# guodashun/peg-in-hole-gym

Hardware: AMD Instinct MI355X
Metric: env-steps/sec (higher is better)
Workload: dtype f32

## Files before the change

### include/pih.h

```cpp
#ifndef PIH_H
#define PIH_H
#include <stdint.h>
#ifdef __cplusplus
extern "C" {
#endif

#define PIH_ABI_VERSION 4
#define PIH_STATE_WORDS 256
#define PIH_ACTION_DIM 4
#define PIH_OBS_DIM 5
#define PIH_DEBUG_WORDS 1024

enum {
  PIH_DBG_UDOT = 0,
  PIH_DBG_NCONTACT = 38,
  PIH_DBG_PGS_ITERS = 39,
  PIH_DBG_CONTACT = 40,
  PIH_DBG_CONTACT_STRIDE = 12,
  PIH_DBG_CONTACT_KEY = 10,
  PIH_DBG_CONTACT_LAMBDA = 11,
  PIH_DBG_DINV = 640,
  PIH_DBG_FLY_UDOT = 0,
  PIH_DBG_FLY_NCONTACT = 12,
  PIH_DBG_FLY_PGS_ITERS = 13,
  PIH_DBG_FLY_LIMIT_ROWS = 14,
  PIH_DBG_FLY_CAND = 16,
  PIH_DBG_FLY_CAND_STRIDE = 10,
  PIH_DBG_FLY_LAMBDA = 200,
  PIH_DBG_CYCLES = 900,
  PIH_DBG_T_START = 940,
  PIH_DBG_T_END = 943,
  PIH_DBG_HW_ID = 946,
  PIH_DBG_XCC_ID = 947
};

enum {
// ... 117 lines not shown
```

### peg_in_hole_gym_amd/_lib.py

```python
import ctypes as C
import os

_HERE = os.path.dirname(os.path.abspath(__file__))
LIB_PATH = os.environ.get("PIH_LIB_PATH") or os.path.join(_HERE, "csrc", "libpih_hip.so")

ABI_VERSION = 4
STATE_WORDS, DEBUG_WORDS, ACTION_DIM, OBS_DIM = 256, 1024, 4, 5
FLY_STATE_WORDS, FLY_ACTION_DIM, FLY_OBS_DIM = 48, 6, 6
CAM_WORDS = 13
FLY_CAM_DEFAULT = (1.6, 0.0, 1.2, 0.0, 0.0, 0.2, 0.0, 0.0, 1.0, 60.0, 1.0, 0.01, 100.0)
RENDER_SHADED, RENDER_CAM_EE = 1, 2
RENDER_OUT_RGBA8, RENDER_OUT_DEPTH, RENDER_CAM_DEVICE = 4, 8, 16
SEG_OBJECT, SEG_TABLE, SEG_NONE = 6, 7, 255
RENDER_CAM_EE_POS = 32
VIEW_SEG_HOLE, VIEW_SEG_TABLE, VIEW_SEG_PIPE0 = 9, 10, 32
VIEW_CAM_WRIST = (0.0, 0.0, 0.0, 0.0, 0.0, -10.0, 0.0, 1.0, 0.0, 60.0, 1.0, 0.001, 1000.0)
VIEW_CAM_OVERVIEW = (1.33, -0.02, 1.05, 0.05, -0.25, 0.3, 0.0, 0.0, 1.0, 40.0, 1.0, 0.01, 100.0)
LIGHT_WORDS = 11
LIGHT_DEFAULT = (-50.0, 30.0, 100.0, 1.0, 1.0, 1.0, 0.6, 0.35, 0.05, 2.0, 0.8)
RENDER_LIGHT_DEVICE = 64
FIELD_STATE, FIELD_TIP_POSE, FIELD_CONTACT_FORCE, FIELD_DEBUG, FIELD_EE_POS = 0, 1, 2, 3, 4
TASK_PEG_IN_HOLE, TASK_RANDOM_FLY = 0, 1
S_QARM, S_QDARM, S_POS, S_QUAT, S_VLIN, S_VANG, S_QJ, S_QDJ, S_TARGET = 0, 9, 18, 21, 25, 28, 31, 54, 77
S_FSM, S_FSMT, S_DONE, S_GRASP, S_RANDY, S_RNG_HI, S_RNG, S_STEPS, S_OFFSET = 86, 87, 88, 89, 90, 91, 92, 93, 94
S_SPARE, S_TIP, S_CFORCE, S_NCONTACT, S_PGS_ITERS, S_EE, S_GRASP_ANGLE, S_INVALID, S_ATTACH_QZ, S_SOLVER = 97, 98, 105, 106, 107, 108, 111, 112, 113, 114
S_CACHE_N, S_CACHE_KEY, S_CACHE_LAMBDA = 128, 129, 177
F_Q, F_QD, F_TARGET, F_OPOS, F_OQUAT, F_OVLIN, F_OVANG, F_DONE, F_STEPS, F_RNG, F_RNG_HI, F_OFFSET, F_SPARE, F_INVALID, F_EE, F_CFORCE, F_NCONTACT = \
    0, 6, 12, 18, 21, 25, 28, 31, 32, 33, 34, 35, 38, 39, 40, 43, 44
DBG_UDOT, DBG_NCONTACT, DBG_PGS_ITERS, DBG_CONTACT, DBG_CONTACT_STRIDE, DBG_CONTACT_KEY, DBG_CONTACT_LAMBDA, DBG_DINV = 0, 38, 39, 40, 12, 10, 11, 640
DBG_FLY_UDOT, DBG_FLY_NCONTACT, DBG_FLY_PGS_ITERS, DBG_FLY_LIMIT_ROWS, DBG_FLY_CAND, DBG_FLY_CAND_STRIDE, DBG_FLY_LAMBDA = 0, 12, 13, 14, 16, 10, 200
DBG_CYCLES, DBG_T_START, DBG_T_END, DBG_HW_ID, DBG_XCC_ID = 900, 940, 943, 946, 947

EXPORTS = ["pih_default_config", "pih_abi_version", "pih_task_dims", "pih_object_name", "pih_create", "pih_destroy", "pih_reset", "pih_reseed", "pih_step", "pih_step_n",
           "pih_get_state", "pih_set_state", "pih_ik", "pih_ik_ur5", "pih_render", "pih_render_ex", "pih_render_cam", "pih_grasp_labels", "pih_timing", "pih_timing2", "pih_set_timing", "pih_last_error"]
LIGHT_EXPORTS = ["pih_render_lit"]
VIEW_EXPORTS = ["pih_render_view"]


class PihConfig(C.Structure):
    _fields_ = [("n_envs", C.c_int32), ("env_index0", C.c_int32), ("mode", C.c_int32), ("solver_iters", C.c_int32),
                ("ik_iters", C.c_int32), ("max_episode_steps", C.c_int32), ("auto_reset", C.c_int32),
                ("enable_self_collision", C.c_int32), ("debug", C.c_int32), ("schedule", C.c_int32), ("enable_arm_collision", C.c_int32), ("task_id", C.c_int32), ("solver_path", C.c_int32), ("attach_ball", C.c_int32), ("exit_check_stride", C.c_int32), ("object_id", C.c_int32), ("seed", C.c_uint64),
                ("dt", C.c_float), ("residual_threshold", C.c_float), ("erp", C.c_float), ("warmstart", C.c_float),
                ("contact_margin", C.c_float), ("linear_slop", C.c_float), ("ik_damping", C.c_float), ("ik_residual", C.c_float),
# ... 79 lines not shown
```

### peg_in_hole_gym_amd/csrc/pih_common.h

```cpp
#pragma once
#include <string.h>
#include "../../include/pih.h"
#include "../../include/pih_model.h"
#include "pih_math.h"

namespace pih {

constexpr int NL = PIH_NL, ANL = PIH_ARM_NL, ONL = PIH_OBJ_NL, ND = PIH_NDOF;
constexpr int NSAMP = PIH_PIPE_NSAMP;
constexpr int CMAX = 48;
constexpr int CAMAX = 12;
constexpr int CL = 20;
constexpr int NROWC = 3 * CMAX;
constexpr int WPS = 39;
constexpr int WMS = 31;
constexpr int NMOT = 32;
constexpr int NLIM = 18;
static_assert(PIH_DBG_UDOT + ND <= PIH_DBG_NCONTACT && PIH_DBG_CONTACT + PIH_DBG_CONTACT_STRIDE * CMAX <= PIH_DBG_DINV &&
              PIH_DBG_DINV + 3 * CMAX <= PIH_DBG_CYCLES && PIH_DBG_XCC_ID < PIH_DEBUG_WORDS, "debug words of the peg-in-hole step (include/pih.h PIH_DBG_*) overlap");

PIH_CONST int L_PARENT[NL] = PIH_LINK_PARENT;
PIH_CONST int L_JTYPE[NL] = PIH_LINK_JTYPE;
PIH_CONST real L_RFIX[NL][9] = PIH_LINK_RFIX;
PIH_CONST real L_TFIX[NL][3] = PIH_LINK_TFIX;
PIH_CONST real L_AXIS[NL][3] = PIH_LINK_AXIS;
PIH_CONST real L_MASS[NL] = PIH_LINK_MASS;
PIH_CONST real L_COM[NL][3] = PIH_LINK_COM;
PIH_CONST real L_INERTIA[NL][6] = PIH_LINK_INERTIA;
PIH_CONST real L_LO[NL] = PIH_LINK_LO;
PIH_CONST real L_HI[NL] = PIH_LINK_HI;
PIH_CONST real L_DAMPING[NL] = PIH_LINK_DAMPING;
PIH_CONST real L_MU[NL] = PIH_LINK_MU;
PIH_CONST real ARM_BASE_R[9] = PIH_ARM_BASE_R;
namespace model_ce {
// ... 54 lines not shown
};

inline void config_defaults(pih_config* c) {
  memset(c, 0, sizeof *c);
  c->n_envs = 1; c->env_index0 = 0; c->mode = 0; c->solver_iters = 50; c->ik_iters = 20; c->max_episode_steps = 2227; c->auto_reset = 0;
  c->enable_self_collision = 1; c->enable_arm_collision = 3; c->task_id = PIH_TASK_PEG_IN_HOLE; c->debug = 0; c->schedule = 1; c->exit_check_stride = 16;
  c->seed = 0; c->dt = 1.0f / 240.0f; c->residual_threshold = 1e-7f; c->erp = 0.2f; c->warmstart = 0.85f; c->contact_margin = 0.005f;
  c->linear_slop = 1e-5f; c->ik_damping = 0.5f; c->ik_residual = 1e-4f; c->dv = 2.0f / 240.0f;
}
inline Params params_from_config(const pih_config* c) {
  Params P;
  P.dt = (real)c->dt; P.resid = (real)c->residual_threshold; P.erp = (real)c->erp; P.warm = (real)c->warmstart; P.margin = (real)c->contact_margin;
  P.slop = (real)c->linear_slop; P.ikdamp = (real)c->ik_damping; P.ikres = (real)c->ik_residual; P.dv = (real)c->dv;
  P.iters = c->solver_iters; P.ikiters = c->ik_iters; P.mode = c->mode; P.maxsteps = c->max_episode_steps; P.autoreset = c->auto_reset;
  P.selfcol = c->enable_self_collision; P.armcol = c->enable_arm_collision; P.debug = c->debug; P.env0 = c->env_index0; P.seed = c->seed;
  P.pgsmode = c->solver_path; P.attachball = c->attach_ball; P.noprio = (c->schedule & 4) != 0; P.nospec = (c->schedule & 64) != 0;
  P.checkstride = c->exit_check_stride < 1 ? 1 : c->exit_check_stride; P.object = c->object_id;
  return P;
}

template <bool DOUBLED = true, class FC, class FN> PIH_HD int pgs_iteration_loop(int iters, int stride, FC checked, FN unchecked) {
  int it = 0;
  const int lead = stride <= 1 ? iters : 4;
  while (it < iters && it < lead) { it++; if (checked()) return it; }
  while (it < iters) {
    const int stop = it + stride - 1 < iters - 1 ? it + stride - 1 : iters - 1;
    if (DOUBLED) {
      while (it < stop) {
        it++; unchecked();
        if (it >= stop) break;
        it++; unchecked();
// ... 837 lines not shown
```

### peg_in_hole_gym_amd/csrc/pih_fly.h

```cpp
#pragma once
#include <type_traits>
#include "pih_common.h"

namespace pih {
namespace fly {

constexpr int NJ = 6, FND = 12, NS = PIH_FLY_OBJ_MAXSPH;
constexpr int NA = 5;
constexpr int NC = 2 * NS + NA;
constexpr int SW = PIH_FLY_STATE_WORDS;
static_assert(PIH_DBG_FLY_UDOT + FND <= PIH_DBG_FLY_NCONTACT && PIH_DBG_FLY_CAND + PIH_DBG_FLY_CAND_STRIDE * NC <= PIH_DBG_FLY_LAMBDA &&
              PIH_DBG_FLY_LAMBDA + NC <= PIH_DBG_CYCLES, "debug words of the random-fly step (include/pih.h PIH_DBG_FLY_*) overlap");
constexpr int CW = 24;
enum : int {
  FC_J = 0,
  FC_W = 6,
  FC_N = 12,
  FC_RXN = 15,
  FC_IRXN = 18,
  FC_DINV = 21,
  FC_RHS = 22,
  FC_LAM = 23,
};
static_assert(FC_W == FC_J + NJ && FC_N == FC_W + NJ && FC_LAM + 1 == CW, "contact row record of the lane layout");
// ... 372 lines not shown
    stamp(4);
    real du[FND], lam_m[NJ], lam_lo[NJ], lam_hi[NJ], wjj[NJ];
    real du3[3], Wq[NJ][3];
#pragma unroll
    for (int j = 0; j < NJ; j++) {
      wjj[j] = Wm[j][j];
#pragma unroll
      for (int k = 0; k < 3; k++) {
        if constexpr (Q::QUAD) Wq[j][k] = quad.lane4() == 0 ? Wm[j][k] : quad.lane4() == 1 ? Wm[j][3 + k] : (real)0;
      }
    }
    const real LIMIT_REACH = (real)0.25;
    int limmask = 0;
#pragma unroll
    for (int j = 0; j < NJ; j++) if (q[j] - U_LO[j] < LIMIT_REACH || U_HI[j] - q[j] < LIMIT_REACH) limmask |= 1 << j;
    limmask = P.nospec ? (1 << NJ) - 1 : quad.wave_or(limmask);
    real viol = -1, vlo[NJ], vhi[NJ];
    auto joint_tot = [&](auto JTAG, real duj, auto CHECKTAG, real& worst) __attribute__((always_inline)) -> real {
      constexpr int j = decltype(JTAG)::value;
      constexpr bool CHECK = decltype(CHECKTAG)::value;
      const real lim = U_EFFORT[j] * dt, di = mdi[j];
      real dl = mrhs[j] - duj * di, sum = med3_(lam_m[j] + dl, -lim, lim);
      dl = sum - lam_m[j]; lam_m[j] = sum;
      if (CHECK) { const real v = dl * dl - P.resid * di * di; worst = v > worst ? v : worst; }
      real dj = duj + dl * wjj[j], tot = dl;
      viol = max_(viol, max_(vlo[j] - dj, dj - vhi[j]));
      if (__builtin_expect(((limmask >> j) & 1) != 0, 0)) {
        const real r2 = lrl[j] - dj * di;
        real s2 = max_(lam_lo[j] + r2, (real)0);
        const real d2 = s2 - lam_lo[j]; lam_lo[j] = s2; tot += d2; dj += d2 * wjj[j];
        if (CHECK) { const real v = d2 * d2 - P.resid * di * di; worst = v > worst ? v : worst; }
// ... 181 lines not shown
```

### peg_in_hole_gym_amd/csrc/pih_hip.hip

```cpp
#include <hip/hip_runtime.h>
#include <dlfcn.h>
#include <cstdio>
#include <cstring>
#include <string>
#include <vector>
#include "pih_device.h"
#include "pih_render.h"
#include "pih_fly.h"
#include "pih_fly_render.h"

using namespace pih;

namespace pih {
void fly_image_launch(int fmt, dim3 grid, hipStream_t stream, const float* state, void* out, const fly::FlyCam& cam, const float* cam_dev,
                      int n, int object, int env_begin, int W, int H, int rows_per_strip, int flags);
void view_launch(int fmt, dim3 grid, hipStream_t stream, const float* state, void* out, const fly::FlyCam& cam, const float* cam_dev,
                 int env_begin, int W, int H, int rows_per_strip, int flags);
int lit_light_check(const float* words, const char** what);
void lit_launch(bool fly_task, int fmt, dim3 grid, hipStream_t stream, const float* state, void* out, const fly::FlyCam& cam, const float* cam_dev,
                const float* light, const float* light_dev, int n, int object, int env_begin, int W, int H, int rows_per_strip, int flags);
}

constexpr int PRE_THREADS = 256;
__device__ __forceinline__ int contact_bin(float ncontact) {
// ... 561 lines not shown
      HIPCHK(h, hipMemset(h->bins, 0, 3 * h->bin_ints * sizeof(int)));
    }
  } else if (cfg->schedule & 1) HIPCHK(h, hipMalloc(&h->order, (size_t)cfg->n_envs * sizeof(int)));
  hipLaunchKernelGGL(pih_init_offsets_kernel, dim3((cfg->n_envs + 63) / 64), dim3(64), 0, 0, h->state, *offd, cfg->n_envs);
  hipLaunchKernelGGL(pih_reset_kernel, dim3(cfg->n_envs), dim3(64), 0, 0, h->P, h->state, (const unsigned char*)nullptr, 0, 0);
  if (h->bins) hipLaunchKernelGGL(pih_bins_init_kernel, dim3(64), dim3(256), 0, 0, h->state, h->bins + h->bin_ints, cfg->n_envs);
  HIPCHK(h, hipGetLastError());
  HIPCHK(h, hipDeviceSynchronize());
  return 0;
}

int pih_create(const pih_config* cfg, const float* offsets_host, pih_handle** out) {
  if (!cfg || !out || cfg->n_envs <= 0) { g_err = "pih_create: bad arguments"; return -2; }
  if (cfg->task_id != PIH_TASK_PEG_IN_HOLE && cfg->task_id != PIH_TASK_RANDOM_FLY) { g_err = "pih_create: unknown task_id"; return -2; }
  if (cfg->task_id == PIH_TASK_RANDOM_FLY && (cfg->object_id < 0 || cfg->object_id >= PIH_FLY_NOBJ)) { g_err = "pih_create: unknown object_id for the random-fly task"; return -2; }
  if ((cfg->schedule & 3) >= 2 || (cfg->schedule & ~(3 | 4 | 8 | 32 | 64)) != 0) {
    g_err = "pih_create: schedule = " + std::to_string(cfg->schedule) + " is not supported (0 or 1, plus any of 4, 8, 32, 64)";
    return -2;
  }
  int ndev = 0;
  hipError_t e = hipGetDeviceCount(&ndev);
  if (e != hipSuccess || ndev == 0) { g_err = "pih_create: no HIP device (this library has no CPU path)"; return -3; }
  pih_handle* h = new pih_handle;
  h->cfg = *cfg; h->P = params_from_config(cfg);
  h->fly = cfg->task_id == PIH_TASK_RANDOM_FLY; h->words = h->fly ? PIH_FLY_STATE_WORDS : PIH_STATE_WORDS;
  float* offd = nullptr;
  int rc = -1;
  if (hipGetDevice(&h->device) == hipSuccess) rc = create_impl(h, offsets_host, &offd);
  else g_err = "pih_create: hipGetDevice failed";
  if (offd) hipFree(offd);
  if (rc != 0) { pih_destroy(h); return rc; }
  *out = h;
// ... 325 lines not shown
```

### peg_in_hole_gym_amd/csrc/pih_step.h

```cpp
#pragma once

namespace pih {

template <class W> PIH_HD void aba(W& w, Shared& sh) {
  w.stamp(15);
  link_velocities(w, sh);
  w.stamp(8);
  w.par(NL, [&](int L) {
    int p = L_PARENT[L], jt = L_JTYPE[L];
    real m = L_MASS[L];
    V3 rc = ld3(sh.a.LRC[L]); S3 Ic = lds3(sh.a.LIC[L]);
    V3 wv = ld3(sh.VW[L]), vv = ld3(sh.VV[L]);
    real* I = sh.a.IAP[L];
    real r2 = dot(rc, rc);
    I[0] = Ic.xx + m * (r2 - rc.x * rc.x); I[1] = Ic.yy + m * (r2 - rc.y * rc.y); I[2] = Ic.zz + m * (r2 - rc.z * rc.z);
    I[3] = Ic.xy - m * rc.x * rc.y; I[4] = Ic.xz - m * rc.x * rc.z; I[5] = Ic.yz - m * rc.y * rc.z;
    I[6] = 0; I[7] = -m * rc.z; I[8] = m * rc.y; I[9] = m * rc.z; I[10] = 0; I[11] = -m * rc.x; I[12] = -m * rc.y; I[13] = m * rc.x; I[14] = 0;
    I[15] = m; I[16] = m; I[17] = m; I[18] = 0; I[19] = 0; I[20] = 0;
    V3 ca = mk(0, 0, 0), cl = mk(0, 0, 0), r = mk(0, 0, 0);
    if (jt != PIH_JT_FLOATING && p >= 0) {
      V3 wp = ld3(sh.VW[p]); r = ld3(sh.LO[L]) - ld3(sh.LO[p]);
      V3 aq = sh.u[link_dof(L)] * ld3(sh.LA[L]);
      cl = cross(wp, cross(wp, r));
      if (jt == PIH_JT_REVOLUTE) ca = cross(wp, aq); else cl = cl + (real)2 * cross(wp, aq);
// ... 48 lines not shown
      if (k == ANL - 3) arm6 = na;
    }
    for (int L = 2 * ANL + 1; L < NL; L++) {
      const OC c = np_c;
      if (L + 1 < NL) np_c = oconst(L + 1);
      pipe = olink(L, pipe, c);
    }
  }
}

template <class W>
PIH_HD void step_env(W& w, Shared& sh, const Params& P, const Ovf& ov, int env, const real* action, real* obs, real* reward, unsigned char* done, real* dbg) {
  real* S = sh.S;
  const real dt = P.dt;
  w.phase_begin();
  bool frozen = !P.autoreset && S[PIH_S_DONE] != 0;
  fk_all(w, sh);
  w.phase(0);
  if (!frozen) {
    if constexpr (W::controller_inline) controller_targets(S, P, action);
    const bool ctrl_early = P.mode != 0;
    if (ctrl_early) { w.await_controller(sh); controller_rows(w, sh, P); }
    else controller_rows(w, sh, P, 1);
    w.phase(1);
    collide(w, sh, P);
    w.priority(sh.nc);
    w.phase(2);
    w.par(ND, [&](int d) {
      real v;
      if (d < 9) v = S[PIH_S_QDARM + d]; else if (d < 12) v = S[PIH_S_VLIN + d - 9]; else if (d < 15) v = S[PIH_S_VANG + d - 12]; else v = S[PIH_S_QDJ + d - 15];
// ... 87 lines not shown
```

### peg_in_hole_gym_amd/csrc/pih_wave.h

```cpp
#pragma once
#include <type_traits>
#include "pih_common.h"
#include "pih_mailbox.h"

namespace pih {

PIH_HD void debug_store_time(real* dbg, int at, long long t) { dbg[at] = (real)(t & 0xFFFF); dbg[at + 1] = (real)((t >> 16) & 0xFFFF); dbg[at + 2] = (real)((t >> 32) & 0xFFFF); }
PIH_HD void debug_store_hw_id(real* dbg) { dbg[PIH_DBG_HW_ID] = (real)(__builtin_amdgcn_s_getreg((15 << 11) | 4) & 0xFFFF); dbg[PIH_DBG_XCC_ID] = (real)__builtin_amdgcn_s_getreg((3 << 11) | 20); }

struct Wave {
  int l;
  int counter;
  static constexpr bool controller_inline = false;
  real* dbg = nullptr; int dbgmode = 0; long long t0 = 0, t1 = 0;
  PIH_HD void stamp(int k) { if (dbg && dbgmode == 2) { long long t = __builtin_readcyclecounter(); if (l == 0) dbg[PIH_DBG_CYCLES + k] = (real)(t - t0); t0 = t; } }
  PIH_HD void trace(int at, long long t) { if (l != 0) return; debug_store_time(dbg, at, t); if (at == PIH_DBG_T_START) debug_store_hw_id(dbg); }
  PIH_HD void phase_begin() { if (dbg && dbgmode == 2) { t1 = __builtin_readcyclecounter(); trace(PIH_DBG_T_START, (long long)__builtin_amdgcn_s_memrealtime()); } }
  PIH_HD void phase(int k) { if (dbg && dbgmode == 2) { long long t = __builtin_readcyclecounter(); if (l == 0) dbg[PIH_DBG_CYCLES + k] = (real)(t - t1); t1 = t; if (k == 7) trace(PIH_DBG_T_END, (long long)__builtin_amdgcn_s_memrealtime()); } }
  PIH_HD int lane() const { return l; }
  bool prio_on = true;
  PIH_HD void priority(int contacts) {
    if (!prio_on) return;
    if (contacts > 20) __builtin_amdgcn_s_setprio(3);
    else if (contacts > 14) __builtin_amdgcn_s_setprio(2);
// ... 46 lines not shown
  __asm__ volatile("v_max_f32 %0, %6, %7\n\tv_sub_f32 %1, %0, %3\n\tv_readlane_b32 %2, %0, %9\n\tv_readlane_b32 s100, %1, %9\n\t"
                   "s_lshl_b64 %4, 1, %9\n\tv_cndmask_b32_e64 %3, %3, %0, %4\n\tv_pk_fma_f32 %5, s[100:101], %8, %5 op_sel_hi:[0,1,1]"
                   : "=&v"(cand), "=&v"(dl), "=&s"(s0), "+v"(lam), "=&s"(m), "+v"(zz) : "v"(z), "v"(lo), "v"(col), "n"(G) : "scc", "s100", "s101");
}
PIH_HD void gs_row2_bounded(pk2& zz, real z, pk2 col, real hi, real& lam, int G, real& dl) {
  real cand; unsigned long long m;
  __asm__ volatile("v_med3_f32 %0, %5, -%6, %6\n\tv_sub_f32 %1, %0, %2\n\ts_lshl_b64 %3, 1, %8\n\tv_readlane_b32 s100, %1, %8\n\t"
                   "v_cndmask_b32_e64 %2, %2, %0, %3\n\ts_nop 0\n\tv_pk_fma_f32 %4, s[100:101], %7, %4 op_sel_hi:[0,1,1]"
                   : "=&v"(cand), "=&v"(dl), "+v"(lam), "=&s"(m), "+v"(zz) : "v"(z), "v"(hi), "v"(col), "n"(G) : "scc", "s100", "s101");
}
PIH_HD void gs_row2_friction(pk2& zz, real z, pk2 col, real h, real& lam, int G, real& dl) {
  real cand; unsigned long long m;
  __asm__ volatile("v_med3_f32 %0, %5, -%6, %6\n\tv_sub_f32 %1, %0, %2\n\ts_lshl_b64 %3, 1, %8\n\tv_readlane_b32 s100, %1, %8\n\t"
                   "v_cndmask_b32_e64 %2, %2, %0, %3\n\ts_nop 0\n\tv_pk_fma_f32 %4, s[100:101], %7, %4 op_sel_hi:[0,1,1]"
                   : "=&v"(cand), "=&v"(dl), "+v"(lam), "=&s"(m), "+v"(zz) : "v"(z), "v"(h), "v"(col), "n"(G) : "scc", "s100", "s101");
}
PIH_HD void gs_row1_normal(real& z, real b, real lo, real& lam, int G, real& dl, real& s0) {
  real cand, sdl; unsigned long long m;
  __asm__ volatile("v_max_f32 %0, %6, %7\n\tv_sub_f32 %1, %0, %4\n\tv_readlane_b32 %3, %0, %9\n\tv_readlane_b32 %2, %1, %9\n\t"
                   "s_lshl_b64 %5, 1, %9\n\tv_cndmask_b32_e64 %4, %4, %0, %5\n\tv_fmac_f32 %6, %2, %8"
                   : "=&v"(cand), "=&v"(dl), "=&s"(sdl), "=&s"(s0), "+v"(lam), "=&s"(m), "+v"(z) : "v"(lo), "v"(b), "n"(G) : "scc");
}
PIH_HD void gs_row1_friction2(real& z, real b1, real b2, real h, real& lam, int G1, int G2, real& dl1, real& dl2) {
  real cand, sdl; unsigned long long m;
  __asm__ volatile("v_med3_f32 %0, %6, -%7, %7\n\tv_sub_f32 %1, %0, %4\n\ts_lshl_b64 %5, 1, %10\n\tv_readlane_b32 %3, %1, %10\n\t"
                   "v_cndmask_b32_e64 %4, %4, %0, %5\n\ts_nop 0\n\tv_fmac_f32 %6, %3, %8\n\t"
                   "v_med3_f32 %0, %6, -%7, %7\n\tv_sub_f32 %2, %0, %4\n\ts_lshl_b64 %5, 1, %11\n\tv_readlane_b32 %3, %2, %11\n\t"
                   "v_cndmask_b32_e64 %4, %4, %0, %5\n\ts_nop 0\n\tv_fmac_f32 %6, %3, %9"
                   : "=&v"(cand), "=&v"(dl1), "=&v"(dl2), "=&s"(sdl), "+v"(lam), "=&s"(m), "+v"(z) : "v"(h), "v"(b1), "v"(b2), "n"(G1), "n"(G2) : "scc");
}
// ... 160 lines not shown
                   "v_add_f32_dpp %1, %1, %1 row_bcast:31 row_mask:0xc\n\t"
                   "v_add_f32_dpp %2, %2, %2 row_bcast:31 row_mask:0xc\n\t"
                   "s_nop 1"
                   : "+v"(a), "+v"(b), "+v"(c));
}
PIH_HD void row16_sum3(real& a, real& b, real& c) {
  a = dpp_add<0xB1>(a); b = dpp_add<0xB1>(b); c = dpp_add<0xB1>(c);
  a = dpp_add<0x4E>(a); b = dpp_add<0x4E>(b); c = dpp_add<0x4E>(c);
  a = dpp_add<0x141>(a); b = dpp_add<0x141>(b); c = dpp_add<0x141>(c);
  a = dpp_add<0x140>(a); b = dpp_add<0x140>(b); c = dpp_add<0x140>(c);
}


template <int W> PIH_HD real rec4(const real4* q) { constexpr int c = W % 4; return c == 0 ? q[W / 4].x : c == 1 ? q[W / 4].y : c == 2 ? q[W / 4].z : q[W / 4].w; }
template <int W> PIH_HD V3 rec4v(const real4* q) { return mk(rec4<W>(q), rec4<W + 1>(q), rec4<W + 2>(q)); }
constexpr int FR = NMOT + 3 * MERGED_CONTACTS;
PIH_HD int pgs_rows(Wave& w, Shared& sh, const Params& P) {
  const int nc = __builtin_amdgcn_readfirstlane(sh.nc);
  w.sync();
  const int lane = w.lane();
  const bool hasarm = __builtin_amdgcn_readfirstlane(sh.nca) != 0;
  real J[ND];
  {
    const bool ismotor = lane < NMOT;
    const int row = ismotor ? 0 : lane - NMOT, c = row / 3, k = row - 3 * c;
    const bool live = !ismotor && c < nc;
    int la = -1, lb = -1; V3 p = mk(0, 0, 0), dir = mk(0, 0, 0); bool ang = false;
    if (live) { la = sh.c_la[c]; lb = sh.c_lb[c]; const real* R = sh.b.crec[c]; p = ld3(R + CR_P); dir = ld3(R + CR_DIR0 + CR_KSTRIDE * k); ang = R[CR_ANG] != 0; }
    const int md = lane < 9 ? lane : 15 + (lane - 9);
    if (!hasarm) {
// ... 49 lines not shown
  else {
    const int row = lane - NMOT, c = row / 3, k = row - 3 * c;
    if (c < nc) {
      const real* R = sh.b.crec[c];
      di = R[CR_DINV0 + CR_KSTRIDE * k]; rhs = R[CR_RHS + k]; thr = R[CR_THRESH + k]; cmu = R[CR_MU]; cfl = R[CR_FLOOR];
      if (k == 0) { lbv = R[CR_LB]; ubv = PIH_BIG; lam0 = sh.r_lam[3 * c]; }
    }
  }
#pragma unroll
  for (int i = 0; i < FR; i++) { A[i] = (lane == i && lane >= 9 ? (real)1 : (real)0) - di * A[i]; }
  real* const Bn = A;
  unsigned angmask = 0;
#pragma unroll
  for (int c = 0; c < MERGED_CONTACTS; c++) if (c < nc && sh.b.crec[c][CR_MU] < 0) angmask |= 1u << c;
  angmask = (unsigned)__builtin_amdgcn_readfirstlane((int)angmask);
  bool skip7 = true;
  {
    const real dt = P.dt;
#pragma unroll
    for (int j = 0; j < 7; j++) {
      const real q = sh.S[PIH_S_QARM + j], uj = sh.u[j];
      const real vt = sh.mrec[j][MR_RHS] * sh.lrec[j][LR_JW] + uj;
      const real plo = q - L_LO[j], phi = L_HI[j] - q;
      const real vlo = plo > 0 ? -plo / dt : -P.erp * plo / dt, vhi = phi > 0 ? -phi / dt : -P.erp * phi / dt;
      const real tol = (real)1e-4 * ((real)1 + absr(vt) + absr(uj) + absr(vlo) + absr(vhi));
      skip7 = skip7 && (vt - vlo > tol) && (-vhi - vt > tol);
    }
    skip7 = skip7 && sh.mrec[0][MR_IMP] >= (real)100;
    skip7 = __builtin_amdgcn_readfirstlane((int)skip7) != 0;
  }
  real armlim = sh.mrec[0][MR_IMP];
#pragma unroll
  for (int j = 1; j < 7; j++) armlim = sh.mrec[j][MR_IMP] < armlim ? sh.mrec[j][MR_IMP] : armlim;
  if (lane < 9) sh.lrec[lane][LR_JWDINV] = sh.lrec[lane][LR_JW] * sh.mrec[lane][MR_DINV];
  w.sync();
  real ind[NMOT];
  real bown = 0;
  const bool spec = __builtin_amdgcn_readfirstlane((int)P.nospec) == 0;
  if (spec) {
#pragma unroll
    for (int g = 0; g < NMOT; g++) {
      if (g == 7 || g == 8) { ind[g] = 0; continue; }
      const bool own = lane == g;
      ind[g] = own ? (real)1 : (real)0;
      if (g >= 9) { bown = own ? Bn[g] : bown; Bn[g] -= ind[g]; }
      __asm__ volatile("" : "+v"(ind[g]));
    }
  } else {
#pragma unroll
    for (int g = 0; g < NMOT; g++) ind[g] = 0;
  }
  real lam_a[9], lam_lo[9], lam_hi[9], lamr[NMOT];
  real lam = 0, z = 0;
// ... 153 lines not shown
  w.sync();
  return it;
}

PIH_HD int pgs_rows2(Wave& w, Shared& sh, const Params& P, const Ovf& ov, const MotorW& mw) {
  const int nc = __builtin_amdgcn_readfirstlane(sh.nc);
  w.sync();
  const int lane = w.lane();
  constexpr int D = 12;
  real* const Bg = ov.base + OVF_B_OFF + 2 * lane;
  static_assert(OVF_MW_WORDS + OVF_PAD_WORDS >= D * 128, "the ring reads D columns past the streamed-column area");
  const unsigned l8 = (unsigned)lane * 8u;
  struct RowC { real di, rhs, thr, lb, ub, mu, fl, lam0; };
  auto rowconst = [&](int g) __attribute__((always_inline)) -> RowC {
    RowC r; r.di = 0; r.rhs = 0; r.thr = PIH_BIG; r.lb = 0; r.ub = 0; r.mu = 0; r.fl = 0; r.lam0 = 0;
    if (g < 9) r.di = sh.mrec[g][MR_DINV];
    else if (g < NMOT) { r.di = sh.mrec[g][MR_DINV]; r.rhs = sh.mrec[g][MR_RHS]; r.thr = sh.mrec[g][MR_THRESH]; r.ub = sh.mrec[g][MR_IMP]; r.lb = -r.ub; }
    else {
      const int row = g - NMOT, c = row / 3, k = row - 3 * c;
      if (c < nc) {
        const real* R = crec_of(sh, ov, c);
        r.di = R[CR_DINV0 + CR_KSTRIDE * k]; r.rhs = R[CR_RHS + k]; r.thr = R[CR_THRESH + k]; r.mu = R[CR_MU]; r.fl = R[CR_FLOOR];
        if (k == 0) { r.lb = R[CR_LB]; r.ub = PIH_BIG; r.lam0 = sh.r_lam[3 * c]; }
      }
    }
    return r;
  };
  const RowC c0 = rowconst(lane), c1 = rowconst(64 + lane);
  pk2 BB[KREG];
  {
    const int row0 = lane - NMOT, row1 = 32 + lane;
// ... 84 lines not shown
      column(cb, [&](int o) __attribute__((always_inline)) { return pk_pack(wr[o], wr[o + 1]); });
    }
    typedef const real __attribute__((address_space(1)))* grp;
#pragma unroll 1
    for (int cb = CL; cb < nc; cb++) {
      const grp wr = (grp)(ov.base + (size_t)(3 * (cb - CL)) * WPS);
      column(cb, [&](int o) __attribute__((always_inline)) { return pk_pack(wr[o], wr[o + 1]); });
    }
  }
#pragma unroll
  for (int q = NMOT; q < KREG; q++) if (q >= NMOT + 3 * nc) BB[q] = 0;
  unsigned angmask = 0;
  for (int c = 0; c < nc; c++) { const real* R = crec_of(sh, ov, c); if (R[CR_MU] < 0) angmask |= 1u << c; }
  angmask = (unsigned)__builtin_amdgcn_readfirstlane((int)angmask);
  if (lane < 9) sh.lrec[lane][LR_JWDINV] = sh.lrec[lane][LR_JW] * sh.mrec[lane][MR_DINV];
  __threadfence_block();
  w.sync();
  real lam0 = c0.lam0, lam1 = c1.lam0, z0, z1;
  real lam_a[9], lam_lo[9], lam_hi[9];
#pragma unroll
  for (int j = 0; j < 9; j++) { lam_a[j] = 0; lam_lo[j] = 0; lam_hi[j] = 0; }
  z0 = c0.rhs + wv0; z1 = c1.rhs + wv1;
  auto iterate = [&](auto CHECKTAG, auto WELDTAG) __attribute__((always_inline)) -> bool {
    constexpr bool CHECK = decltype(CHECKTAG)::value;
    constexpr bool WELD = decltype(WELDTAG)::value;
    unsigned long long busy = 0;
    __asm__ volatile("" ::: "memory");
    typedef const char __attribute__((address_space(1)))* gcp;
    typedef const pk2 __attribute__((address_space(1)))* gpp;
    gcp colp = (gcp)(ov.base + OVF_B_OFF);
    __asm__ volatile("" : "+s"(colp));
    auto ldcol = [&](int sidx) __attribute__((always_inline)) -> pk2 { return *(gpp)(colp + (size_t)sidx * 512 + l8); };
    pk2 rr[D];
#pragma unroll
    for (int s = 0; s < D; s++) rr[s] = ldcol(s);
    constexpr int PF = 2;
    real4 pa4[PF], pl4[PF];
#pragma unroll
    for (int k = 0; k < PF; k++) { pa4[k] = *reinterpret_cast<const real4*>(sh.mrec[k]); pl4[k] = *reinterpret_cast<const real4*>(sh.lrec[k]); }
    real za = z0; pk2 zp1 = pk_pack(z0, z1);
#pragma unroll
    for (int j = 0; j < PIH_OBJ_NJ; j++) {
      if (j < 9) {
        const real4 ca = pa4[j % PF], cl = pl4[j % PF];
        if (j + PF < 9) { pa4[j % PF] = *reinterpret_cast<const real4*>(sh.mrec[j + PF]); pl4[j % PF] = *reinterpret_cast<const real4*>(sh.lrec[j + PF]); }
        const real rh = rec4<MR_RHS>(&ca), th = rec4<MR_THRESH>(&ca), lim = rec4<MR_IMP>(&ca);
        const real lor = rec4<LR_LO>(&cl), hir = rec4<LR_HI>(&cl), wd = rec4<LR_JWDINV>(&cl);
        real y = -rdlane(za, j);
        real sum = lam_a[j] + (rh - y);
        sum = med3_(sum, -lim, lim);
        const real dl = sum - lam_a[j]; lam_a[j] = sum;
        if (CHECK) busy |= __ballot(absr(dl) > th);
        y += dl * wd;
        real s2 = lam_lo[j] + (lor - y); s2 = max_(s2, (real)0);
        const real d2 = s2 - lam_lo[j]; lam_lo[j] = s2;
        if (CHECK) busy |= __ballot(absr(d2) > th);
        y += d2 * wd;
        real s3 = lam_hi[j] + (hir + y); s3 = max_(s3, (real)0);
        const real d3 = s3 - lam_hi[j]; lam_hi[j] = s3;
        if (CHECK) busy |= __ballot(absr(d3) > th);
        const real tot = dl + d2 - d3;
        za += pk_lo(BB[j]) * tot; zp1 = pk_pack(pk_lo(zp1), pk_hi(zp1) + pk_hi(BB[j]) * tot);
      }
      const int g = 9 + j;
      real dlv;
      gs_row2_bounded(zp1, pk_lo(zp1), BB[g], c0.ub, lam0, g, dlv);
      if (CHECK) busy |= __ballot(absr(dlv) > c0.thr) & (1ull << g);
    }
    pk2 zz = pk_pack((za + pk_lo(zp1)) - z0, pk_hi(zp1));
    int ncl = nc; unsigned am = angmask;
    unsigned l8c = l8;
    gcp colq = colp + D * 512;
    __asm__ volatile("" : "+s"(colq));
#pragma unroll
    for (int c = 0; c < HC; c++) {
      __asm__ volatile("" : "+s"(ncl), "+s"(am), "+v"(l8c));
      if (c >= ncl) break;
      const int g0 = NMOT + 3 * c;
      pk2 bb[3];
#pragma unroll
      for (int k = 0; k < 3; k++) {
        const int sc = g0 + k - KREG;
        bb[k] = rr[sc % D];
        rr[sc % D] = *(gpp)(colq + ((c & 1) * 3 + k) * 512 + l8c);
// ... 6 lines not shown
      if (g0 < 64) { gs_row2_normal(zz, pk_lo(zz), bb[0], c0.lb, lam0, g0, dl, s0); if (CHECK) busy |= __ballot(absr(dl) > c0.thr) & (1ull << g0); }
      else { gs_row2_normal(zz, pk_hi(zz), bb[0], c1.lb, lam1, g0 - 64, dl, s0); if (CHECK) busy |= __ballot(absr(dl) > c1.thr) & (1ull << (g0 - 64)); }
      const int s0i = __builtin_bit_cast(int, s0), weld = WELD ? (int)((am >> c) & 1u) : 0;
      if (WELD ? (s0i > weld ? s0i : weld) > 0 : s0i > 0) {
        auto friction = [&](int g, pk2 col) __attribute__((always_inline)) {
          if (g < 64) { const real h0 = max_(c0.mu * s0, c0.fl); gs_row2_friction(zz, pk_lo(zz), col, h0, lam0, g, dl); if (CHECK) busy |= __ballot(absr(dl) > c0.thr) & (1ull << g); }
          else { const real h1 = max_(c1.mu * s0, c1.fl); gs_row2_friction(zz, pk_hi(zz), col, h1, lam1, g - 64, dl); if (CHECK) busy |= __ballot(absr(dl) > c1.thr) & (1ull << (g - 64)); }
        };
        friction(g0 + 1, bb[1]);
        friction(g0 + 2, bb[2]);
      }
    }
    z0 = pk_lo(zz); z1 = pk_hi(zz);
    return CHECK && busy == 0;
  };
  int it;
  if (angmask != 0) it = pgs_iteration_loop<false>(P.iters, P.checkstride, [&]() __attribute__((always_inline)) { return iterate(std::true_type{}, std::true_type{}); }, [&]() __attribute__((always_inline)) { return iterate(std::false_type{}, std::true_type{}); });
  else it = pgs_iteration_loop<false>(P.iters, P.checkstride, [&]() __attribute__((always_inline)) { return iterate(std::true_type{}, std::false_type{}); }, [&]() __attribute__((always_inline)) { return iterate(std::false_type{}, std::false_type{}); });
  if (lane == 0) sh.S[PIH_S_SOLVER] = 5;
  if (lane >= NMOT && lane < NMOT + 3 * nc) sh.r_lam[lane - NMOT] = lam0;
  if (32 + lane < 3 * nc) sh.r_lam[32 + lane] = lam1;
  if (lane >= 9 && lane < NMOT) sh.mrec[lane][MR_LAM] = lam0;
#pragma unroll
  for (int j = 0; j < 9; j++) if (lane == 0) sh.mrec[j][MR_LAM] = lam_a[j] + lam_lo[j] - lam_hi[j];
  w.sync();
  {
    const int d = lane, dw = d < ND ? d : ND;
    real du = 0;
#pragma unroll
    for (int j = 0; j < PIH_OBJ_NJ; j++) {
      du += Mg[j * 64] * (d < 9 ? (j < 9 ? sh.mrec[j][MR_LAM] : (real)0) : sh.mrec[9 + j][MR_LAM]);
    }
    {
// ... 168 lines not shown
```

Baseline: 11.78 million.

## Add speculative unbounded-residual PGS form for the two-row solver with fallback

Adds a speculative solver form for the rows2 PGS path when no weld contacts are present. Motor rows are treated as unbounded residual updates, and the arm limit rows are skipped entirely when the arm limits are provably idle. The iteration state is parked in unused response rows beforehand. After the solve, the multipliers are checked against the motor bounds, and if any bound is exceeded the solve reruns with the original clamped form. This removes the per-row clamp and limit work on the common path, at the cost of a full re-solve when the speculation fails, plus extra register and code-size pressure.

```diff
diff --git a/include/pih.h b/include/pih.h
--- a/include/pih.h
+++ b/include/pih.h
@@ -20,6 +20,7 @@
   PIH_DBG_CONTACT_KEY = 10,
   PIH_DBG_CONTACT_LAMBDA = 11,
   PIH_DBG_DINV = 640,
+  PIH_DBG_ROWS2_FORM = 800,
   PIH_DBG_FLY_UDOT = 0,
   PIH_DBG_FLY_NCONTACT = 12,
   PIH_DBG_FLY_PGS_ITERS = 13,
diff --git a/peg_in_hole_gym_amd/_lib.py b/peg_in_hole_gym_amd/_lib.py
--- a/peg_in_hole_gym_amd/_lib.py
+++ b/peg_in_hole_gym_amd/_lib.py
@@ -27,7 +27,7 @@
 S_CACHE_N, S_CACHE_KEY, S_CACHE_LAMBDA = 128, 129, 177
 F_Q, F_QD, F_TARGET, F_OPOS, F_OQUAT, F_OVLIN, F_OVANG, F_DONE, F_STEPS, F_RNG, F_RNG_HI, F_OFFSET, F_SPARE, F_INVALID, F_EE, F_CFORCE, F_NCONTACT = \
     0, 6, 12, 18, 21, 25, 28, 31, 32, 33, 34, 35, 38, 39, 40, 43, 44
-DBG_UDOT, DBG_NCONTACT, DBG_PGS_ITERS, DBG_CONTACT, DBG_CONTACT_STRIDE, DBG_CONTACT_KEY, DBG_CONTACT_LAMBDA, DBG_DINV = 0, 38, 39, 40, 12, 10, 11, 640
+DBG_UDOT, DBG_NCONTACT, DBG_PGS_ITERS, DBG_CONTACT, DBG_CONTACT_STRIDE, DBG_CONTACT_KEY, DBG_CONTACT_LAMBDA, DBG_DINV, DBG_ROWS2_FORM = 0, 38, 39, 40, 12, 10, 11, 640, 800
 DBG_FLY_UDOT, DBG_FLY_NCONTACT, DBG_FLY_PGS_ITERS, DBG_FLY_LIMIT_ROWS, DBG_FLY_CAND, DBG_FLY_CAND_STRIDE, DBG_FLY_LAMBDA = 0, 12, 13, 14, 16, 10, 200
 DBG_CYCLES, DBG_T_START, DBG_T_END, DBG_HW_ID, DBG_XCC_ID = 900, 940, 943, 946, 947
 
diff --git a/peg_in_hole_gym_amd/csrc/pih_common.h b/peg_in_hole_gym_amd/csrc/pih_common.h
--- a/peg_in_hole_gym_amd/csrc/pih_common.h
+++ b/peg_in_hole_gym_amd/csrc/pih_common.h
@@ -17,7 +17,7 @@
 constexpr int NMOT = 32;
 constexpr int NLIM = 18;
 static_assert(PIH_DBG_UDOT + ND <= PIH_DBG_NCONTACT && PIH_DBG_CONTACT + PIH_DBG_CONTACT_STRIDE * CMAX <= PIH_DBG_DINV &&
-              PIH_DBG_DINV + 3 * CMAX <= PIH_DBG_CYCLES && PIH_DBG_XCC_ID < PIH_DEBUG_WORDS, "debug words of the peg-in-hole step (include/pih.h PIH_DBG_*) overlap");
+              PIH_DBG_DINV + 3 * CMAX <= PIH_DBG_ROWS2_FORM && PIH_DBG_ROWS2_FORM < PIH_DBG_CYCLES && PIH_DBG_XCC_ID < PIH_DEBUG_WORDS, "debug words of the peg-in-hole step (include/pih.h PIH_DBG_*) overlap");
 
 PIH_CONST int L_PARENT[NL] = PIH_LINK_PARENT;
 PIH_CONST int L_JTYPE[NL] = PIH_LINK_JTYPE;
@@ -102,7 +102,7 @@
   P.slop = (real)c->linear_slop; P.ikdamp = (real)c->ik_damping; P.ikres = (real)c->ik_residual; P.dv = (real)c->dv;
   P.iters = c->solver_iters; P.ikiters = c->ik_iters; P.mode = c->mode; P.maxsteps = c->max_episode_steps; P.autoreset = c->auto_reset;
   P.selfcol = c->enable_self_collision; P.armcol = c->enable_arm_collision; P.debug = c->debug; P.env0 = c->env_index0; P.seed = c->seed;
-  P.pgsmode = c->solver_path; P.attachball = c->attach_ball; P.noprio = (c->schedule & 4) != 0; P.nospec = (c->schedule & 64) != 0;
+  P.pgsmode = c->solver_path; P.attachball = c->attach_ball; P.noprio = (c->schedule & 4) != 0; P.nospec = ((c->schedule & 64) != 0 ? 1 : 0) | ((c->schedule & 256) != 0 ? 2 : 0);
   P.checkstride = c->exit_check_stride < 1 ? 1 : c->exit_check_stride; P.object = c->object_id;
   return P;
 }
diff --git a/peg_in_hole_gym_amd/csrc/pih_fly.h b/peg_in_hole_gym_amd/csrc/pih_fly.h
--- a/peg_in_hole_gym_amd/csrc/pih_fly.h
+++ b/peg_in_hole_gym_amd/csrc/pih_fly.h
@@ -410,7 +410,7 @@
     int limmask = 0;
 #pragma unroll
     for (int j = 0; j < NJ; j++) if (q[j] - U_LO[j] < LIMIT_REACH || U_HI[j] - q[j] < LIMIT_REACH) limmask |= 1 << j;
-    limmask = P.nospec ? (1 << NJ) - 1 : quad.wave_or(limmask);
+    limmask = (P.nospec & 1) ? (1 << NJ) - 1 : quad.wave_or(limmask);
     real viol = -1, vlo[NJ], vhi[NJ];
     auto joint_tot = [&](auto JTAG, real duj, auto CHECKTAG, real& worst) __attribute__((always_inline)) -> real {
       constexpr int j = decltype(JTAG)::value;
diff --git a/peg_in_hole_gym_amd/csrc/pih_hip.hip b/peg_in_hole_gym_amd/csrc/pih_hip.hip
--- a/peg_in_hole_gym_amd/csrc/pih_hip.hip
+++ b/peg_in_hole_gym_amd/csrc/pih_hip.hip
@@ -599,8 +599,8 @@
   if (!cfg || !out || cfg->n_envs <= 0) { g_err = "pih_create: bad arguments"; return -2; }
   if (cfg->task_id != PIH_TASK_PEG_IN_HOLE && cfg->task_id != PIH_TASK_RANDOM_FLY) { g_err = "pih_create: unknown task_id"; return -2; }
   if (cfg->task_id == PIH_TASK_RANDOM_FLY && (cfg->object_id < 0 || cfg->object_id >= PIH_FLY_NOBJ)) { g_err = "pih_create: unknown object_id for the random-fly task"; return -2; }
-  if ((cfg->schedule & 3) >= 2 || (cfg->schedule & ~(3 | 4 | 8 | 32 | 64)) != 0) {
-    g_err = "pih_create: schedule = " + std::to_string(cfg->schedule) + " is not supported (0 or 1, plus any of 4, 8, 32, 64)";
+  if ((cfg->schedule & 3) >= 2 || (cfg->schedule & ~(3 | 4 | 8 | 32 | 64 | 256)) != 0) {
+    g_err = "pih_create: schedule = " + std::to_string(cfg->schedule) + " is not supported (0 or 1, plus any of 4, 8, 32, 64, 256)";
     return -2;
   }
   int ndev = 0;
diff --git a/peg_in_hole_gym_amd/csrc/pih_step.h b/peg_in_hole_gym_amd/csrc/pih_step.h
--- a/peg_in_hole_gym_amd/csrc/pih_step.h
+++ b/peg_in_hole_gym_amd/csrc/pih_step.h
@@ -86,6 +86,7 @@
   real* S = sh.S;
   const real dt = P.dt;
   w.phase_begin();
+  if (dbg && P.debug) dbg[PIH_DBG_ROWS2_FORM] = 0;
   bool frozen = !P.autoreset && S[PIH_S_DONE] != 0;
   fk_all(w, sh);
   w.phase(0);
diff --git a/peg_in_hole_gym_amd/csrc/pih_wave.h b/peg_in_hole_gym_amd/csrc/pih_wave.h
--- a/peg_in_hole_gym_amd/csrc/pih_wave.h
+++ b/peg_in_hole_gym_amd/csrc/pih_wave.h
@@ -84,6 +84,17 @@
   __asm__ volatile("v_med3_f32 %0, %5, -%6, %6\n\tv_sub_f32 %1, %0, %2\n\ts_lshl_b64 %3, 1, %8\n\tv_readlane_b32 s100, %1, %8\n\t"
                    "v_cndmask_b32_e64 %2, %2, %0, %3\n\ts_nop 0\n\tv_pk_fma_f32 %4, s[100:101], %7, %4 op_sel_hi:[0,1,1]"
                    : "=&v"(cand), "=&v"(dl), "+v"(lam), "=&s"(m), "+v"(zz) : "v"(z), "v"(h), "v"(col), "n"(G) : "scc", "s100", "s101");
+}
+PIH_HD void gs_row2_residual(pk2& zz, real r, pk2 col, real& lam, int G) {
+  real t; unsigned long long m;
+  __asm__ volatile("s_lshl_b64 %2, 1, %6\n\tv_readlane_b32 s100, %4, %6\n\tv_add_f32 %0, %1, %4\n\tv_cndmask_b32_e64 %1, %1, %0, %2\n\t"
+                   "v_pk_fma_f32 %3, s[100:101], %5, %3 op_sel_hi:[0,1,1]"
+                   : "=&v"(t), "+v"(lam), "=&s"(m), "+v"(zz) : "v"(r), "v"(col), "n"(G) : "scc", "s100", "s101");
+}
+PIH_HD real rdlane_after_block(real v, int G) {
+  real s;
+  __asm__ volatile("s_nop 0\n\tv_readlane_b32 %0, %1, %2\n\ts_nop 1" : "=s"(s) : "v"(v), "n"(G));
+  return s;
 }
 PIH_HD void gs_row1_normal(real& z, real b, real lo, real& lam, int G, real& dl, real& s0) {
   real cand, sdl; unsigned long long m;
@@ -274,6 +285,31 @@
 
 template <int W> PIH_HD real rec4(const real4* q) { constexpr int c = W % 4; return c == 0 ? q[W / 4].x : c == 1 ? q[W / 4].y : c == 2 ? q[W / 4].z : q[W / 4].w; }
 template <int W> PIH_HD V3 rec4v(const real4* q) { return mk(rec4<W>(q), rec4<W + 1>(q), rec4<W + 2>(q)); }
+PIH_HD real arm_motor_bound(Shared& sh) {
+  real armlim = sh.mrec[0][MR_IMP];
+#pragma unroll
+  for (int j = 1; j < 7; j++) armlim = sh.mrec[j][MR_IMP] < armlim ? sh.mrec[j][MR_IMP] : armlim;
+  return armlim;
+}
+PIH_HD bool arm_limit_rows_idle(Shared& sh, const Params& P, real& armlim) {
+  bool skip7 = true;
+  {
+    const real dt = P.dt;
+#pragma unroll
+    for (int j = 0; j < 7; j++) {
+      const real q = sh.S[PIH_S_QARM + j], uj = sh.u[j];
+      const real vt = sh.mrec[j][MR_RHS] * sh.lrec[j][LR_JW] + uj;
+      const real plo = q - L_LO[j], phi = L_HI[j] - q;
+      const real vlo = plo > 0 ? -plo / dt : -P.erp * plo / dt, vhi = phi > 0 ? -phi / dt : -P.erp * phi / dt;
+      const real tol = (real)1e-4 * ((real)1 + absr(vt) + absr(uj) + absr(vlo) + absr(vhi));
+      skip7 = skip7 && (vt - vlo > tol) && (-vhi - vt > tol);
+    }
+    skip7 = skip7 && sh.mrec[0][MR_IMP] >= (real)100;
+    skip7 = __builtin_amdgcn_readfirstlane((int)skip7) != 0;
+  }
+  armlim = arm_motor_bound(sh);
+  return skip7;
+}
 constexpr int FR = NMOT + 3 * MERGED_CONTACTS;
 PIH_HD int pgs_rows(Wave& w, Shared& sh, const Params& P) {
   const int nc = __builtin_amdgcn_readfirstlane(sh.nc);
@@ -353,29 +389,13 @@
 #pragma unroll
   for (int c = 0; c < MERGED_CONTACTS; c++) if (c < nc && sh.b.crec[c][CR_MU] < 0) angmask |= 1u << c;
   angmask = (unsigned)__builtin_amdgcn_readfirstlane((int)angmask);
-  bool skip7 = true;
-  {
-    const real dt = P.dt;
-#pragma unroll
-    for (int j = 0; j < 7; j++) {
-      const real q = sh.S[PIH_S_QARM + j], uj = sh.u[j];
-      const real vt = sh.mrec[j][MR_RHS] * sh.lrec[j][LR_JW] + uj;
-      const real plo = q - L_LO[j], phi = L_HI[j] - q;
-      const real vlo = plo > 0 ? -plo / dt : -P.erp * plo / dt, vhi = phi > 0 ? -phi / dt : -P.erp * phi / dt;
-      const real tol = (real)1e-4 * ((real)1 + absr(vt) + absr(uj) + absr(vlo) + absr(vhi));
-      skip7 = skip7 && (vt - vlo > tol) && (-vhi - vt > tol);
-    }
-    skip7 = skip7 && sh.mrec[0][MR_IMP] >= (real)100;
-    skip7 = __builtin_amdgcn_readfirstlane((int)skip7) != 0;
-  }
-  real armlim = sh.mrec[0][MR_IMP];
-#pragma unroll
-  for (int j = 1; j < 7; j++) armlim = sh.mrec[j][MR_IMP] < armlim ? sh.mrec[j][MR_IMP] : armlim;
+  real armlim;
+  const bool skip7 = arm_limit_rows_idle(sh, P, armlim);
   if (lane < 9) sh.lrec[lane][LR_JWDINV] = sh.lrec[lane][LR_JW] * sh.mrec[lane][MR_DINV];
   w.sync();
   real ind[NMOT];
   real bown = 0;
-  const bool spec = __builtin_amdgcn_readfirstlane((int)P.nospec) == 0;
+  const bool spec = (__builtin_amdgcn_readfirstlane((int)P.nospec) & 1) == 0;
   if (spec) {
 #pragma unroll
     for (int g = 0; g < NMOT; g++) {
@@ -559,7 +579,7 @@
   struct RowC { real di, rhs, thr, lb, ub, mu, fl, lam0; };
   auto rowconst = [&](int g) __attribute__((always_inline)) -> RowC {
     RowC r; r.di = 0; r.rhs = 0; r.thr = PIH_BIG; r.lb = 0; r.ub = 0; r.mu = 0; r.fl = 0; r.lam0 = 0;
-    if (g < 9) r.di = sh.mrec[g][MR_DINV];
+    if (g < 9) { r.di = sh.mrec[g][MR_DINV]; if (g < 7) r.thr = sh.mrec[g][MR_THRESH]; }
     else if (g < NMOT) { r.di = sh.mrec[g][MR_DINV]; r.rhs = sh.mrec[g][MR_RHS]; r.thr = sh.mrec[g][MR_THRESH]; r.ub = sh.mrec[g][MR_IMP]; r.lb = -r.ub; }
     else {
       const int row = g - NMOT, c = row / 3, k = row - 3 * c;
@@ -674,16 +694,33 @@
   for (int c = 0; c < nc; c++) { const real* R = crec_of(sh, ov, c); if (R[CR_MU] < 0) angmask |= 1u << c; }
   angmask = (unsigned)__builtin_amdgcn_readfirstlane((int)angmask);
   if (lane < 9) sh.lrec[lane][LR_JWDINV] = sh.lrec[lane][LR_JW] * sh.mrec[lane][MR_DINV];
+  real lam0 = c0.lam0, lam1 = c1.lam0;
+  real z0 = c0.rhs + wv0, z1 = c1.rhs + wv1;
+  const bool spec = (__builtin_amdgcn_readfirstlane((int)P.nospec) & 2) == 0 && angmask == 0;
+  bool skip7 = false;
+  static_assert(3 * (CMAX - HC) * WPS >= 5 * 64, "the parked restart values fit the unused response rows");
+  real* const Pk = ov.base + (size_t)3 * (HC - CL) * WPS + lane;
+  if (spec) {
+    real armlim0;
+    skip7 = arm_limit_rows_idle(sh, P, armlim0);
+    real bown = 0;
+#pragma unroll
+    for (int g = 9; g < NMOT; g++) {
+      const bool own = lane == g;
+      const real b = pk_lo(BB[g]);
+      bown = own ? b : bown;
+      BB[g] = pk_pack(b - (own ? (real)1 : (real)0), pk_hi(BB[g]));
+    }
+    Pk[0] = bown; Pk[64] = z0; Pk[128] = z1; Pk[192] = lam0; Pk[256] = lam1;
+  }
   __threadfence_block();
   w.sync();
-  real lam0 = c0.lam0, lam1 = c1.lam0, z0, z1;
   real lam_a[9], lam_lo[9], lam_hi[9];
-#pragma unroll
-  for (int j = 0; j < 9; j++) { lam_a[j] = 0; lam_lo[j] = 0; lam_hi[j] = 0; }
-  z0 = c0.rhs + wv0; z1 = c1.rhs + wv1;
-  auto iterate = [&](auto CHECKTAG, auto WELDTAG) __attribute__((always_inline)) -> bool {
+  real wmax = 0;
+  auto iterate = [&](auto CHECKTAG, auto WELDTAG, auto FORMTAG) __attribute__((always_inline)) -> bool {
     constexpr bool CHECK = decltype(CHECKTAG)::value;
     constexpr bool WELD = decltype(WELDTAG)::value;
+    constexpr int FORM = decltype(FORMTAG)::value;
     unsigned long long busy = 0;
     __asm__ volatile("" ::: "memory");
     typedef const char __attribute__((address_space(1)))* gcp;
@@ -697,16 +734,23 @@
     constexpr int PF = 2;
     real4 pa4[PF], pl4[PF];
 #pragma unroll
-    for (int k = 0; k < PF; k++) { pa4[k] = *reinterpret_cast<const real4*>(sh.mrec[k]); pl4[k] = *reinterpret_cast<const real4*>(sh.lrec[k]); }
+    for (int k = 0; k < PF; k++) {
+      const int j = FORM == 2 ? 7 + (k + 1) % PF : k;
+      pa4[k] = *reinterpret_cast<const real4*>(sh.mrec[j]); pl4[k] = *reinterpret_cast<const real4*>(sh.lrec[j]);
+    }
+    static_assert(PF == 2, "form 2 loads the records of joints 7 and 8 into slots 7 % PF and 8 % PF");
     real za = z0; pk2 zp1 = pk_pack(z0, z1);
 #pragma unroll
     for (int j = 0; j < PIH_OBJ_NJ; j++) {
-      if (j < 9) {
+      if (FORM == 2 && j < 7) {
+        if (CHECK) busy |= __ballot(absr(pk_lo(zp1)) > c0.thr) & (1ull << j);
+        gs_row2_residual(zp1, pk_lo(zp1), BB[j], lam0, j);
+      } else if (j < 9) {
         const real4 ca = pa4[j % PF], cl = pl4[j % PF];
-        if (j + PF < 9) { pa4[j % PF] = *reinterpret_cast<const real4*>(sh.mrec[j + PF]); pl4[j % PF] = *reinterpret_cast<const real4*>(sh.lrec[j + PF]); }
+        if (FORM != 2 && j + PF < 9) { pa4[j % PF] = *reinterpret_cast<const real4*>(sh.mrec[j + PF]); pl4[j % PF] = *reinterpret_cast<const real4*>(sh.lrec[j + PF]); }
         const real rh = rec4<MR_RHS>(&ca), th = rec4<MR_THRESH>(&ca), lim = rec4<MR_IMP>(&ca);
         const real lor = rec4<LR_LO>(&cl), hir = rec4<LR_HI>(&cl), wd = rec4<LR_JWDINV>(&cl);
-        real y = -rdlane(za, j);
+        real y = FORM == 2 ? -rdlane_after_block(pk_lo(zp1), j) : -rdlane(za, j);
         real sum = lam_a[j] + (rh - y);
         sum = med3_(sum, -lim, lim);
         const real dl = sum - lam_a[j]; lam_a[j] = sum;
@@ -720,14 +764,21 @@
         const real d3 = s3 - lam_hi[j]; lam_hi[j] = s3;
         if (CHECK) busy |= __ballot(absr(d3) > th);
         const real tot = dl + d2 - d3;
-        za += pk_lo(BB[j]) * tot; zp1 = pk_pack(pk_lo(zp1), pk_hi(zp1) + pk_hi(BB[j]) * tot);
+        if (FORM == 2) zp1 = pk_pack(pk_lo(zp1) + pk_lo(BB[j]) * tot, pk_hi(zp1) + pk_hi(BB[j]) * tot);
+        else { za += pk_lo(BB[j]) * tot; zp1 = pk_pack(pk_lo(zp1), pk_hi(zp1) + pk_hi(BB[j]) * tot); }
       }
       const int g = 9 + j;
-      real dlv;
-      gs_row2_bounded(zp1, pk_lo(zp1), BB[g], c0.ub, lam0, g, dlv);
-      if (CHECK) busy |= __ballot(absr(dlv) > c0.thr) & (1ull << g);
-    }
-    pk2 zz = pk_pack((za + pk_lo(zp1)) - z0, pk_hi(zp1));
+      if (FORM == 0) {
+        real dlv;
+        gs_row2_bounded(zp1, pk_lo(zp1), BB[g], c0.ub, lam0, g, dlv);
+        if (CHECK) busy |= __ballot(absr(dlv) > c0.thr) & (1ull << g);
+      } else {
+        if (CHECK) busy |= __ballot(absr(pk_lo(zp1)) > c0.thr) & (1ull << g);
+        gs_row2_residual(zp1, pk_lo(zp1), BB[g], lam0, g);
+      }
+    }
+    if (FORM != 0) wmax = max_(wmax, absr(lam0));
+    pk2 zz = FORM == 2 ? zp1 : pk_pack((za + pk_lo(zp1)) - z0, pk_hi(zp1));
     int ncl = nc; unsigned am = angmask;
     unsigned l8c = l8;
     gcp colq = colp + D * 512;
@@ -764,9 +815,45 @@
     z0 = pk_lo(zz); z1 = pk_hi(zz);
     return CHECK && busy == 0;
   };
-  int it;
-  if (angmask != 0) it = pgs_iteration_loop<false>(P.iters, P.checkstride, [&]() __attribute__((always_inline)) { return iterate(std::true_type{}, std::true_type{}); }, [&]() __attribute__((always_inline)) { return iterate(std::false_type{}, std::true_type{}); });
-  else it = pgs_iteration_loop<false>(P.iters, P.checkstride, [&]() __attribute__((always_inline)) { return iterate(std::true_type{}, std::false_type{}); }, [&]() __attribute__((always_inline)) { return iterate(std::false_type{}, std::false_type{}); });
+  auto zero_arm = [&]() __attribute__((always_inline)) {
+#pragma unroll
+    for (int j = 0; j < 9; j++) { lam_a[j] = 0; lam_lo[j] = 0; lam_hi[j] = 0; }
+  };
+  int it = 0, form = 0;
+  if (spec) {
+    zero_arm();
+    if (skip7) {
+      form = 2;
+      if (lane < 7) z0 += sh.mrec[lane][MR_RHS];
+      it = pgs_iteration_loop<false>(P.iters, P.checkstride, [&]() __attribute__((always_inline)) { return iterate(std::true_type{}, std::false_type{}, std::integral_constant<int, 2>{}); }, [&]() __attribute__((always_inline)) { return iterate(std::false_type{}, std::false_type{}, std::integral_constant<int, 2>{}); });
+    } else {
+      form = 1;
+      it = pgs_iteration_loop<false>(P.iters, P.checkstride, [&]() __attribute__((always_inline)) { return iterate(std::true_type{}, std::false_type{}, std::integral_constant<int, 1>{}); }, [&]() __attribute__((always_inline)) { return iterate(std::false_type{}, std::false_type{}, std::integral_constant<int, 1>{}); });
+    }
+    {
+      const bool resrow = (lane >= 9 && lane < NMOT) || (form == 2 && lane < 7);
+      const real bound = lane < 7 ? arm_motor_bound(sh) : sh.mrec[lane < NMOT ? lane : 0][MR_IMP];
+      const unsigned lb = __builtin_bit_cast(unsigned, bound * (real)0.9921875);
+      const unsigned wb = __builtin_bit_cast(unsigned, wmax), fb = __builtin_bit_cast(unsigned, lam0) & 0x7fffffffu;
+      const bool ok = lb < 0x7f800000u && wb < lb && fb < lb;
+      if (__ballot(resrow && !ok) != 0) {
+        form = 3;
+        const real pb = Pk[0];
+#pragma unroll
+        for (int g = 9; g < NMOT; g++) BB[g] = lane == g ? pk_pack(pb, pk_hi(BB[g])) : BB[g];
+        z0 = Pk[64]; z1 = Pk[128]; lam0 = Pk[192]; lam1 = Pk[256];
+      } else if (form == 2) {
+#pragma unroll
+        for (int j = 0; j < 7; j++) lam_a[j] = rdlane(lam0, j);
+      }
+    }
+  }
+  if (form == 0 || form == 3) {
+    zero_arm();
+    if (angmask != 0) it = pgs_iteration_loop<false>(P.iters, P.checkstride, [&]() __attribute__((always_inline)) { return iterate(std::true_type{}, std::true_type{}, std::integral_constant<int, 0>{}); }, [&]() __attribute__((always_inline)) { return iterate(std::false_type{}, std::true_type{}, std::integral_constant<int, 0>{}); });
+    else it = pgs_iteration_loop<false>(P.iters, P.checkstride, [&]() __attribute__((always_inline)) { return iterate(std::true_type{}, std::false_type{}, std::integral_constant<int, 0>{}); }, [&]() __attribute__((always_inline)) { return iterate(std::false_type{}, std::false_type{}, std::integral_constant<int, 0>{}); });
+  }
+  if (w.dbg && P.debug && lane == 0) w.dbg[PIH_DBG_ROWS2_FORM] = (real)form;
   if (lane == 0) sh.S[PIH_S_SOLVER] = 5;
   if (lane >= NMOT && lane < NMOT + 3 * nc) sh.r_lam[lane - NMOT] = lam0;
   if (32 + lane < 3 * nc) sh.r_lam[32 + lane] = lam1;
```

New measurement: 11.79 million, median of 6. Within noise of the previous version (+0.1%).
